# aurianer/DLA-Future

Hardware: AMD Instinct MI355X
Metric: fp64 Cholesky TFlop/s (higher is better)
Workload: dtype f64; 1 GPU; cholesky_d N=65536 nb=1024 uplo=L; grid=1x1, rank_order=column-major, transport=none, work_copies=5

## Files before the change

dla_future_amd/capi.py:

```python
from __future__ import annotations

import ctypes as C
import os

import numpy as np

_HERE = os.path.dirname(os.path.abspath(__file__))


class LibraryNotBuilt(RuntimeError):
    pass


def lib_path() -> str:
    return os.environ.get("DLAF_MI355X_LIB") or os.path.join(_HERE, "lib", "libdlaf_mi355x.so")


class DLAFDescriptor(C.Structure):
    _fields_ = [("m", C.c_int), ("n", C.c_int), ("mb", C.c_int), ("nb", C.c_int), ("isrc", C.c_int),
                ("jsrc", C.c_int), ("i", C.c_int), ("j", C.c_int), ("ld", C.c_int)]


class UpdateDesc(C.Structure):
    _fields_ = ([(n, C.c_long) for n in ("c_elems", "a_elems", "b_elems", "a2_elems", "b2_elems",
                                         "c_off", "a_off", "b_off", "a2_off", "b2_off")] +
                [("tile_layout", C.c_int), ("ltr", C.c_int), ("ltc", C.c_int),
                 ("c_tsr", C.c_long), ("c_tsc", C.c_long), ("ldc", C.c_int),
                 ("a_ts", C.c_long), ("lda", C.c_int),
                 ("b_ts", C.c_long), ("ldb", C.c_int), ("b_period", C.c_int), ("b_ts2", C.c_long), ("b_jl0", C.c_int)] +
                [(n, C.c_int) for n in ("il0", "il1", "jl0", "jl1", "nb", "K", "pr", "ri", "pc", "ci", "nt", "last_rows",
                                        "rect", "nt_c", "last_cols", "K1", "her2k", "info", "role")] +
                [("max_blocks", C.c_long), ("excl_rounds", C.c_int),
                 ("persistent", C.c_long), ("exclusive", C.c_long), ("bulk_slots", C.c_long)])


class TrsmDesc(C.Structure):
    _fields_ = ([(n, C.c_long) for n in ("b_elems", "l_elems", "w_elems", "b_off", "l_off", "w_off", "b_ts")] +
                [(n, C.c_int) for n in ("ldb", "il0", "il1", "pr", "ri", "nb", "nt", "last_rows", "ldl", "n", "upper",
                                        "prio", "info", "winv_source", "unit", "path", "vec", "info_out")])


class PotrfDesc(C.Structure):
    _fields_ = ([(n, C.c_long) for n in ("t_elems", "w_elems", "t_off", "w_off")] +
                [(n, C.c_int) for n in ("kb", "ld", "info", "info_base", "path", "sync_zeroed_by", "count_strips",
                                        "info_out", "t_before_changed", "w_before_changed")])


BCAST_FN = C.CFUNCTYPE(C.c_int, C.c_void_p, C.c_int, C.c_int, C.c_void_p, C.c_size_t)
BARRIER_FN = C.CFUNCTYPE(C.c_int, C.c_void_p)

_TYPE_CHARS = {np.dtype(np.float32): "s", np.dtype(np.float64): "d", np.dtype(np.complex64): "c",
               np.dtype(np.complex128): "z"}


def type_char(dtype) -> str:
    try:
        return _TYPE_CHARS[np.dtype(dtype)]
    except KeyError:
        raise TypeError(f"unsupported element type {dtype}: expected float32/64 or complex64/128") from None


_vp, _i, _l, _ch = C.c_void_p, C.c_int, C.c_long, C.c_char
_IP = C.POINTER(C.c_int)
_i64 = C.c_int64
_LP = C.POINTER(C.c_long)
SIGNATURES = {
    "dlaf_initialize": (None, [_i, C.POINTER(C.c_char_p), _i, C.POINTER(C.c_char_p)]),
    "dlaf_finalize": (None, []),
    "dlaf_free_grid": (None, [_i]),
    "make_dlaf_descriptor": (DLAFDescriptor, [_i, _i, _i, _i, _IP]),
    "dlaf_cholesky_factorization_s": (_i, [_i, _ch, _vp, DLAFDescriptor]),
    "dlaf_cholesky_factorization_d": (_i, [_i, _ch, _vp, DLAFDescriptor]),
    "dlaf_cholesky_factorization_c": (_i, [_i, _ch, _vp, DLAFDescriptor]),
    "dlaf_cholesky_factorization_z": (_i, [_i, _ch, _vp, DLAFDescriptor]),
    "dlaf_pspotrf": (None, [_ch, _i, _vp, _i, _i, _IP, _IP]),
    "dlaf_pdpotrf": (None, [_ch, _i, _vp, _i, _i, _IP, _IP]),
    "dlaf_pcpotrf": (None, [_ch, _i, _vp, _i, _i, _IP, _IP]),
    "dlaf_pzpotrf": (None, [_ch, _i, _vp, _i, _i, _IP, _IP]),
    "dlaf_mi355x_version": (C.c_char_p, []),
    "dlaf_mi355x_create_grid_single": (_i, []),
    "dlaf_mi355x_rccl_unique_id": (None, [_vp]),
    "dlaf_mi355x_create_grid_rccl": (_i, [_vp, _i, _i, _i, _i, _ch]),
    "dlaf_mi355x_create_grid_host": (_i, [_i, _i, _i, _i, _ch, BCAST_FN, BARRIER_FN, _vp]),
    "dlaf_mi355x_grid_host_bcast": (_i, [_i, _i, _i, _vp, C.c_size_t]),
    "dlaf_mi355x_grid_info": (_i, [_i, _IP, _IP, _IP, _IP]),
    "dlaf_mi355x_grid_barrier": (_i, [_i]),
# ... 302 lines not shown
```

dla_future_amd/csrc/device/mma_core.hpp:

```cpp
#pragma once
#include "common.hpp"

namespace dlaf_mi355x {

template <class T, int BM_, int BN_, int WM_, int WN_, int BK_, bool PAIRED_ = false, int STAGES_ = 2,
          int THREADS_ = kThreads>
struct BlockCfg {
  using R = real_t<T>;
  static constexpr bool CX = TypeInfo<T>::is_complex;
  static constexpr int BM = BM_, BN = BN_, WM = WM_, WN = WN_, BK = BK_;
  static constexpr int THREADS = THREADS_, NWAVES = THREADS_ / 64;
  static constexpr int TM = WM / 16, TN = WN / 16;
  static constexpr int WAVES_M = BM / WM, WAVES_N = BN / WN;
  static_assert(WAVES_M * WAVES_N == NWAVES, "the wave tiles must cover the block");
  static_assert(BK % 4 == 0 && WM % 16 == 0 && WN % 16 == 0, "MFMA 16x16x4 granularity");
  static constexpr bool PAIRED = PAIRED_ && !CX;
  static constexpr bool CXI = PAIRED_ && CX;
  static_assert(!PAIRED || (TM % 2 == 0 && TN % 2 == 0), "paired rows: even tile counts");
  static constexpr int PAD = PAIRED_ ? 0 : kLdsPad;
  static constexpr int LDA = BM + PAD, LDB = BN + PAD;
  static constexpr int EPP = CX ? 64 : 1024 / (int) sizeof(T);
  static constexpr int PIECES_A = BK * BM / EPP, PIECES_B = BK * BN / EPP;
  static constexpr bool GLDS =
      (PAIRED && (EPP % BM == 0 || BM % EPP == 0) && (EPP % BN == 0 || BN % EPP == 0) && (BK * BM) % EPP == 0 &&
       (BK * BN) % EPP == 0 && PIECES_A % NWAVES == 0 && PIECES_B % NWAVES == 0) ||
      (CXI && sizeof(T) == 16 && BM % 64 == 0 && BN % 64 == 0 && PIECES_A % NWAVES == 0 && PIECES_B % NWAVES == 0);
  static constexpr int LPS = PIECES_A / NWAVES + PIECES_B / NWAVES;
  static constexpr int A_PLANE = BK * LDA, B_PLANE = BK * LDB;
  static constexpr int A_ELEMS = (CX ? 2 : 1) * A_PLANE, B_ELEMS = (CX ? 2 : 1) * B_PLANE;
  static constexpr int BUF_ELEMS = A_ELEMS + B_ELEMS;
  static constexpr int STAGES = STAGES_;
  static_assert(STAGES >= 2 && STAGES <= 6, "2..6 LDS stages");
  static constexpr int LDS_BYTES = STAGES * BUF_ELEMS * (int) sizeof(R);
};

template <class Cfg>
struct Acc {
  using R = typename Cfg::R;
  using acc_t = typename Mma<R>::acc_t;
  acc_t re[Cfg::TM][Cfg::TN];
  acc_t im[Cfg::CX ? Cfg::TM : 1][Cfg::CX ? Cfg::TN : 1];

  __device__ __forceinline__ void clear() {
#pragma unroll
    for (int i = 0; i < Cfg::TM; ++i)
#pragma unroll
      for (int j = 0; j < Cfg::TN; ++j) {
        re[i][j] = acc_t{0, 0, 0, 0};
        if constexpr (Cfg::CX)
          im[i][j] = acc_t{0, 0, 0, 0};
      }
  }
};

// ... 188 lines not shown
  if constexpr (Cfg::PAIRED)
    return (j >> 1) * 32 + 2 * Mma<R>::irow(g, v) + (j & 1);
  else
    return j * 16 + Mma<R>::irow(g, v);
}

template <class Cfg, class T>
__device__ __forceinline__ void stage_glds(const T* __restrict__ A, long lda, const T* __restrict__ B, long ldb, int k0,
                                           typename Cfg::R* __restrict__ buf, int wave, int lane) {
  constexpr int NA = Cfg::PIECES_A / Cfg::NWAVES, NB = Cfg::PIECES_B / Cfg::NWAVES;
  constexpr int QA0 = 0, QA1 = NA, QB0 = 0, QB1 = NB;
  if constexpr (Cfg::CXI) {
    constexpr int PA = Cfg::BM / 64, PB = Cfg::BN / 64;
#pragma unroll
    for (int idx = QA0; idx < QA1; ++idx) {
      const int piece = wave + Cfg::NWAVES * idx;
      const int k = piece / PA, part = piece % PA;
      const T* ga = A + part * 64 + lane + (long) (k0 + k) * lda;
      __builtin_amdgcn_global_load_lds((const __attribute__((address_space(1))) void*) ga,
                                       (__attribute__((address_space(3))) void*) (buf + 2 * (k * Cfg::LDA + part * 64)),
                                       16, 0, 0);
    }
#pragma unroll
    for (int idx = QB0; idx < QB1; ++idx) {
      const int piece = wave + Cfg::NWAVES * idx;
      const int k = piece / PB, part = piece % PB;
      const T* gb = B + part * 64 + lane + (long) (k0 + k) * ldb;
      __builtin_amdgcn_global_load_lds(
          (const __attribute__((address_space(1))) void*) gb,
          (__attribute__((address_space(3))) void*) (buf + Cfg::A_ELEMS + 2 * (k * Cfg::LDB + part * 64)), 16, 0, 0);
    }
    return;
  }
  constexpr int PER = 16 / (int) sizeof(T);
  constexpr int EPP = Cfg::EPP;
#pragma unroll
  for (int q = QA0; q < QA1; ++q) {
    const int e0 = (wave * NA + q) * EPP;
    const int e = e0 + lane * PER;
    const T* ga = A + (e % Cfg::BM) + (long) (k0 + e / Cfg::BM) * lda;
    __builtin_amdgcn_global_load_lds((const __attribute__((address_space(1))) void*) ga,
                                     (__attribute__((address_space(3))) void*) (buf + e0), 16, 0, 0);
  }
#pragma unroll
  for (int q = QB0; q < QB1; ++q) {
    const int e0 = (wave * NB + q) * EPP;
    const int e = e0 + lane * PER;
    const T* gb = B + (e % Cfg::BN) + (long) (k0 + e / Cfg::BN) * ldb;
    __builtin_amdgcn_global_load_lds((const __attribute__((address_space(1))) void*) gb,
                                     (__attribute__((address_space(3))) void*) (buf + Cfg::A_ELEMS + e0), 16, 0, 0);
  }
}

template <class Cfg, class T, int IDX>
__device__ __forceinline__ void stage_glds_one(const T* __restrict__ A, long lda, const T* __restrict__ B, long ldb,
                                               int k0, typename Cfg::R* __restrict__ buf, int wave, int lane) {
  static_assert(!Cfg::CXI, "real types");
  constexpr int NA = Cfg::PIECES_A / Cfg::NWAVES, NB = Cfg::PIECES_B / Cfg::NWAVES;
  constexpr int PER = 16 / (int) sizeof(T), EPP = Cfg::EPP;
  auto at = [](const T* base, unsigned byte_off) {
    return reinterpret_cast<const T*>(reinterpret_cast<const char*>(base) + byte_off);
  };
  if constexpr (IDX < NA) {
    static_assert(EPP % Cfg::BM == 0 || Cfg::BM % EPP == 0, "pieces and columns nest");
    const int e0 = (wave * NA + IDX) * EPP;
    const unsigned loff = (unsigned) sizeof(T) * (unsigned) ((lane * PER) % Cfg::BM + ((lane * PER) / Cfg::BM) * (int) lda);
    const T* ga = A + (e0 % Cfg::BM) + (long) (k0 + e0 / Cfg::BM) * lda;
    __builtin_amdgcn_global_load_lds((const __attribute__((address_space(1))) void*) at(ga, loff),
                                     (__attribute__((address_space(3))) void*) (buf + e0), 16, 0, 0);
  }
  else if constexpr (IDX < NA + NB) {
    static_assert(EPP % Cfg::BN == 0 || Cfg::BN % EPP == 0, "pieces and columns nest");
    const int e0 = (wave * NB + (IDX - NA)) * EPP;
    const unsigned loff = (unsigned) sizeof(T) * (unsigned) ((lane * PER) % Cfg::BN + ((lane * PER) / Cfg::BN) * (int) ldb);
    const T* gb = B + (e0 % Cfg::BN) + (long) (k0 + e0 / Cfg::BN) * ldb;
    __builtin_amdgcn_global_load_lds((const __attribute__((address_space(1))) void*) at(gb, loff),
                                     (__attribute__((address_space(3))) void*) (buf + Cfg::A_ELEMS + e0), 16, 0, 0);
  }
}

template <class Cfg, class T, bool VEC, bool EDGE, bool UTAIL = false, bool NEG = false>
__device__ __forceinline__ void gemm_nt_block(const T* __restrict__ A, long lda, int mrows,
                                              const T* __restrict__ B, long ldb, int ncols, int K,
                                              typename Cfg::R* __restrict__ lds, Acc<Cfg>& acc, int K1 = 1 << 30,
                                              const T* __restrict__ A2 = nullptr,
                                              const T* __restrict__ B2 = nullptr, int s0 = 0) {
  using R = typename Cfg::R;
  const int lane = threadIdx.x & 63;
  const int wave = __builtin_amdgcn_readfirstlane(threadIdx.x >> 6);
  const int wm = wave % Cfg::WAVES_M, wn = wave / Cfg::WAVES_M;
  const int nk = (K + Cfg::BK - 1) / Cfg::BK;
  if (nk == 0)
    return;
  if constexpr (Cfg::GLDS && VEC && !EDGE) {
    constexpr int ST = Cfg::STAGES;
    constexpr int LPS = Cfg::LPS;
    static_assert(LPS * (ST - 2) < 64, "vmcnt is a 6-bit counter");
#pragma unroll
    for (int s = 0; s < ST - 1; ++s)
      if (s < nk) {
        int sl = s0 + s;
        sl = sl >= nk ? sl - nk : sl;
        stage_glds<Cfg, T>(sl * Cfg::BK < K1 ? A : A2, lda, sl * Cfg::BK < K1 ? B : B2, ldb, sl * Cfg::BK,
                           lds + s * Cfg::BUF_ELEMS, wave, lane);
      }
    if (nk >= ST - 1)
      __builtin_amdgcn_s_waitcnt(0x0070 | ((LPS * (ST - 2)) & 0xF) | ((((LPS * (ST - 2)) >> 4) & 0x3) << 14));
    else
      asm volatile("s_waitcnt vmcnt(0)" ::: "memory");
    __builtin_amdgcn_s_barrier();
    int cur_i = 0, nxt_i = ST - 1;
    constexpr bool SPLIT = !Cfg::CXI && LPS <= (Cfg::BK / 4) * Cfg::TN && LPS <= 16;
    for (int kt = 0; kt < nk; ++kt) {
      R* cur = lds + cur_i * Cfg::BUF_ELEMS;
      const bool load = UTAIL || (kt + ST - 1 < nk);
      int sn = s0 + min(kt + ST - 1, nk - 1);
      sn = sn >= nk ? sn - nk : sn;
      const int kn = sn * Cfg::BK;
      const T* An = kn < K1 ? A : A2;
      const T* Bn = kn < K1 ? B : B2;
      R* nbuf = lds + nxt_i * Cfg::BUF_ELEMS;
      if constexpr (SPLIT) {
        mma_slab<Cfg, NEG>(cur, cur + Cfg::A_ELEMS, acc, wm, wn, lane, [&](int p) {
#define DLAF_GLDS_AT(I)                                                                     \
  if (p == I) {                                                                           \
    if constexpr (I < LPS)                                                                \
      if (load)                                                                           \
        stage_glds_one<Cfg, T, (I < LPS ? I : 0)>(An, lda, Bn, ldb, kn, nbuf, wave, lane); \
  }
          DLAF_GLDS_AT(0) DLAF_GLDS_AT(1) DLAF_GLDS_AT(2) DLAF_GLDS_AT(3) DLAF_GLDS_AT(4) DLAF_GLDS_AT(5)
          DLAF_GLDS_AT(6) DLAF_GLDS_AT(7) DLAF_GLDS_AT(8) DLAF_GLDS_AT(9) DLAF_GLDS_AT(10) DLAF_GLDS_AT(11)
          DLAF_GLDS_AT(12) DLAF_GLDS_AT(13) DLAF_GLDS_AT(14) DLAF_GLDS_AT(15)
#undef DLAF_GLDS_AT
        });
      }
      else {
        if (load)
          stage_glds<Cfg, T>(An, lda, Bn, ldb, kn, nbuf, wave, lane);
        mma_slab<Cfg, NEG>(cur, cur + Cfg::A_ELEMS, acc, wm, wn, lane);
      }
      if (load)
        __builtin_amdgcn_s_waitcnt(0x0070 | ((LPS * (ST - 2)) & 0xF) | ((((LPS * (ST - 2)) >> 4) & 0x3) << 14));
      else
        asm volatile("s_waitcnt vmcnt(0)" ::: "memory");
      asm volatile("s_waitcnt lgkmcnt(0)" ::: "memory");
      __builtin_amdgcn_s_barrier();
      cur_i = (cur_i + 1 == ST) ? 0 : cur_i + 1;
      nxt_i = (nxt_i + 1 == ST) ? 0 : nxt_i + 1;
    }
    if constexpr (UTAIL) {
      asm volatile("s_waitcnt vmcnt(0)" ::: "memory");
      __builtin_amdgcn_s_barrier();
    }
    return;
  }
  Slab<T, Cfg::BM, Cfg::BK, VEC, Cfg::LDA, Cfg::CXI, Cfg::THREADS> sa;
  Slab<T, Cfg::BN, Cfg::BK, VEC, Cfg::LDB, Cfg::CXI, Cfg::THREADS> sb;
  sa.template load<EDGE>(0 < K1 ? A : A2, lda, 0, mrows, K, A2, K1);
  sb.template load<EDGE>(0 < K1 ? B : B2, ldb, 0, ncols, K, B2, K1);
  sa.store(lds);
  sb.store(lds + Cfg::A_ELEMS);
  __syncthreads();
  for (int kt = 0; kt < nk; ++kt) {
    R* cur = lds + (kt & 1) * Cfg::BUF_ELEMS;
    R* nxt = lds + ((kt + 1) & 1) * Cfg::BUF_ELEMS;
    const bool more = (kt + 1) < nk;
    if (more) {
      const int kn = (kt + 1) * Cfg::BK;
      sa.template load<EDGE>(kn < K1 ? A : A2, lda, kn, mrows, K, A2, K1);
      sb.template load<EDGE>(kn < K1 ? B : B2, ldb, kn, ncols, K, B2, K1);
    }
    mma_slab<Cfg, NEG>(cur, cur + Cfg::A_ELEMS, acc, wm, wn, lane);
    if (more) {
      sa.store(nxt);
      sb.store(nxt + Cfg::A_ELEMS);
    }
    __syncthreads();
  }
}

}
```

dla_future_amd/csrc/host/cholesky.cpp:

```cpp
#include "launch_args.hpp"
#include "runtime.hpp"

#include <algorithm>
#include <cstdlib>
#include <cstring>
#include <vector>

namespace dlaf_mi355x {

static bool potrf_use_chain() {
  static const bool chain = [] {
    const char* e = std::getenv("DLAF_MI355X_POTRF");
    return e && std::strcmp(e, "chain") == 0;
  }();
  return chain;
}

template <class T>
void potrf_tile_coop(T* t, int ld, int kb, T* winv, int* info, int info_base, unsigned* sync, hipStream_t s,
                     bool sync_is_zero, bool count_strips) {
  launch_potrf_coop(t, ld, kb, winv, info, info_base, sync, s, sync_is_zero, count_strips);
}

template <class T>
// ... 76 lines not shown
  const long cap = ncols > 0 ? (ncols + period - 1) / period : 0;
  ts2 = cap * (long) tile_elems;
  int issued = 0;
  tr->group_begin();
  for (long c = 0; c < period && c < ncols; ++c) {
    const long jl_first = jl_n + c;
    const long gj_first = cols.global_of(jl_first);
    const int root_r = rows.owner(gj_first);
    long cnt = (ncols - c + period - 1) / period;
    if (cols.global_of(jl_first + (cnt - 1) * period) == nt - 1)
      --cnt;
    if (cnt <= 0)
      continue;
    T* d = dst + c * ts2;
    if (rows.rank == root_r) {
      const T* src = a_base + (size_t) (rows.local_of(gj_first) - il_n) * tile_elems;
      DLAF_HIP_CHECK(hipMemcpy2DAsync(d, tile_bytes, src, (size_t) lstep * tile_bytes, tile_bytes, (size_t) cnt,
                                      hipMemcpyDeviceToDevice, s));
    }
    tr->bcast(ax_col, root_r, rows.rank, d, d, (size_t) cnt * tile_bytes, s);
    ++issued;
  }
  tr->group_end();
  return issued;
}

namespace {

enum class Schedule { Pairs, Sidecar, Early, Classic };

Schedule choose_schedule(bool dist, int nb, bool complex_type) {
  const char* e = std::getenv("DLAF_MI355X_SCHEDULE");
  if (e == nullptr) {
    if (dist)
      return Schedule::Early;
    if (nb % 16 == 0)
      return Schedule::Pairs;
    return !complex_type && nb <= 768 ? Schedule::Sidecar : Schedule::Classic;
  }
  if (std::strcmp(e, "early") == 0)
    return Schedule::Early;
  if (!dist && std::strcmp(e, "pairs") == 0)
    return Schedule::Pairs;
  if (!dist && std::strcmp(e, "sidecar") == 0)
    return Schedule::Sidecar;
  return Schedule::Classic;
}

constexpr long kSidecarSlots = 32;

template <class T>
struct PairRates {
  static constexpr bool dbl = sizeof(real_t<T>) == 8;
  static constexpr double r_bulk = dbl ? 66e12 : 118e12;
  static constexpr double r_trsm_slot = (dbl ? 5e12 : 8e12) / 32.0;
  static constexpr double t_potrf_blk2 = 11.3e-6 * (TypeInfo<T>::is_complex ? 2.0 : 1.0);
};

template <class T>
struct Step {
  const T* a_base = nullptr;
  const T* b_base = nullptr;
  long b_ts = 0, il_n = 0, jl_n = 0;
  int b_period = 1;
  long b_ts2 = 0;
  const T* a2_base = nullptr;
  const T* b2_base = nullptr;
  int k1 = 0;
  int kb = 0;
  long rest0 = 0, split = 0;
  bool valid = false;

  static Step one_panel(int kb, long il_n, long jl_n, const T* a_base, size_t tile_elems) {
    Step st;
    st.valid = true;
    st.kb = kb;
    st.il_n = il_n;
    st.jl_n = jl_n;
    st.a_base = st.b_base = a_base;
    st.b_ts = (long) tile_elems;
    return st;
  }
  static Step two_panels(int k1, int k2, long n0, const T* a_base, const T* a2_base, size_t tile_elems) {
    Step st = one_panel(k1 + k2, n0, n0, a_base, tile_elems);
    st.k1 = k1;
    st.a2_base = st.b2_base = a2_base;
    return st;
  }
};

template <class T>
struct CholeskyIssue {
  using StepT = Step<T>;
  DeviceMatrix<T>& m;
  Transport* tr;
  const bool dist;
  const size_t tile_bytes;
  const CommAxis ax_row, ax_col;
  const hipStream_t s_main, s_panel, s_comm;
  long potrf_slots = 0, comm_slots = 0;
  long grid_reserve = 0;
  size_t next_update_slice = 0;

  explicit CholeskyIssue(DeviceMatrix<T>& mat)
      : m(mat), tr(grid_transport(*mat.grid)), dist(mat.grid->nranks > 1), tile_bytes(mat.tile_elems * sizeof(T)),
        ax_row(mat.transposed ? CommAxis::Col : CommAxis::Row),
        ax_col(mat.transposed ? CommAxis::Row : CommAxis::Col), s_main(mat.s_low), s_panel(mat.s_high),
// ... 491 lines not shown
```

dla_future_amd/csrc/host/update_direct.cpp:

```cpp
#include <algorithm>
#include <vector>

#include <dlaf_mi355x/dlaf_mi355x.h>

#include "launch_args.hpp"
#include "runtime.hpp"
#include "tile_matrix.hpp"

namespace dlaf_mi355x {

namespace {

template <class T>
struct TileGrid {
  T* tiles;
  size_t tile_elems;
  long ltr, ltc;
  int nb;
  Axis rows, cols;
};

template <class T>
struct Operand {
  DevBuf<T> buf;
  T* p = nullptr;
  void put(const void* host, long elems, long off, hipStream_t s) {
    buf.alloc((size_t) (elems + off));
    p = buf.p + off;
    if (elems > 0)
      DLAF_HIP_CHECK(hipMemcpyAsync(p, host, (size_t) elems * sizeof(T), hipMemcpyHostToDevice, s));
  }
};

template <class T>
bool in_bounds(const UpdateArgs<T>& ua, const dlaf_mi355x_update_desc& d) {
  if (ua.pr < 1 || ua.pc < 1 || ua.ri < 0 || ua.ri >= ua.pr || ua.ci < 0 || ua.ci >= ua.pc || ua.il0 < 0 || ua.jl0 < 0 ||
      ua.nb < 1 || ua.K < 1 || ua.nt < 1 || ua.last_rows < 1 || ua.last_rows > ua.nb || ua.ldc < 1 || ua.lda < 1 ||
      ua.ldb < 1 || ua.b_period < 1 || ua.K1 < 0 || ua.K1 >= ua.K || (ua.her2k && ua.K1 == 0) ||
      (ua.rect && (ua.nt_c < 1 || ua.last_cols < 1 || ua.last_cols > ua.nb)) || (ua.rect && ua.her2k))
    return false;
  const int bj0 = ua.b_jl0 >= 0 ? ua.b_jl0 : ua.jl0;
  if (bj0 > ua.jl0)
    return false;
  const long k2 = ua.K - ua.K1;
  const long ka = ua.K1 > 0 ? (ua.her2k ? std::max<long>(ua.K1, k2) : ua.K1) : ua.K;
  const long ka2 = ua.her2k ? std::max<long>(ua.K1, k2) : k2;
  const long kb = ua.K1 > 0 ? ua.K1 : ua.K;
  auto inside = [](long first, long last, long elems) { return first >= 0 && last < elems; };
  for (long il = ua.il0; il < ua.il1; ++il) {
    const long gi = il * ua.pr + ua.ri;
    if (gi >= ua.nt)
      return false;
    const long rows = gi == ua.nt - 1 ? ua.last_rows : ua.nb;
    if (rows > ua.lda || rows > ua.ldc)
      return false;
    const long a0 = (il - ua.il0) * ua.a_ts;
    bool row_used = false;
    for (long jl = ua.jl0; jl < ua.jl1; ++jl) {
      const long gj = jl * ua.pc + ua.ci;
      if (!ua.rect && gi < gj)
        continue;
      if (gj >= (ua.rect ? ua.nt_c : ua.nt))
        return false;
      row_used = true;
      const long cols = ua.rect ? (gj == ua.nt_c - 1 ? ua.last_cols : ua.nb) : (gj == ua.nt - 1 ? ua.last_rows : ua.nb);
      const long c0 = il * ua.c_tsr + jl * ua.c_tsc;
      if (!inside(c0, c0 + rows - 1 + (cols - 1) * ua.ldc, d.c_elems))
        return false;
      if (!ua.rect && gi == gj)
        continue;
      if (cols > ua.ldb)
        return false;
      const long jt = jl - bj0;
      const long b0 = (jt % ua.b_period) * ua.b_ts2 + (jt / ua.b_period) * ua.b_ts;
      if (!inside(b0, b0 + cols - 1 + (kb - 1) * ua.ldb, d.b_elems))
        return false;
      if (ua.K1 > 0 && !inside(b0, b0 + cols - 1 + (k2 - 1) * ua.ldb, d.b2_elems))
        return false;
    }
    if (!row_used)
      continue;
    if (!inside(a0, a0 + rows - 1 + (ka - 1) * ua.lda, d.a_elems))
      return false;
    if (ua.K1 > 0 && !inside(a0, a0 + rows - 1 + (ka2 - 1) * ua.lda, d.a2_elems))
      return false;
  }
  return true;
}

}

template <class T>
long update_bulk_slots() {
  runtime_init();
  hipDeviceProp_t prop;
  int dev = 0;
  DLAF_HIP_CHECK(hipGetDevice(&dev));
  DLAF_HIP_CHECK(hipGetDeviceProperties(&prop, dev));
  return (long) prop.multiProcessorCount * update_blocks_per_cu<T>();
}

template <class T>
int update_direct(dlaf_mi355x_update_desc& d, void* c, const void* a, const void* b, const void* a2, const void* b2,
                  void* c_again) {
  runtime_init();
  if (d.role < 0 || d.role > 4)
    return -1;
  if (d.c_elems < 1 || d.a_elems < 1 || d.b_elems < 1 || d.c_off < 0 || d.a_off < 0 || d.b_off < 0 || d.a2_off < 0 ||
      d.b2_off < 0 || d.excl_rounds < 0 || (d.K1 > 0 && (d.a2_elems < 1 || d.b2_elems < 1 || !a2 || !b2)))
    return -3;
  hipStream_t s = nullptr;
  Operand<T> dc, da, db, da2, db2;
  dc.put(c, d.c_elems, d.c_off, s);
  da.put(a, d.a_elems, d.a_off, s);
  db.put(b, d.b_elems, d.b_off, s);
  if (d.K1 > 0) {
    da2.put(a2, d.a2_elems, d.a2_off, s);
    db2.put(b2, d.b2_elems, d.b2_off, s);
  }
  DevBuf<int> info(1);
  DevBuf<unsigned> counters(16);
  DLAF_HIP_CHECK(hipMemcpyAsync(info.p, &d.info, sizeof(int), hipMemcpyHostToDevice, s));
  DLAF_HIP_CHECK(hipMemsetAsync(counters.p, 0, 16 * sizeof(unsigned), s));

  UpdateArgs<T> ua{};
  if (d.tile_layout) {
    if (d.ltr < 1 || d.ltc < 1 || d.nb < 1 || d.pr < 1 || d.pc < 1 || d.nt < 1)
      return -3;
    TileGrid<T> m;
    m.tiles = dc.p;
    m.tile_elems = (size_t) d.nb * d.nb;
    m.ltr = d.ltr;
    m.ltc = d.ltc;
    m.nb = d.nb;
    m.rows = Axis{(long) (d.nt - 1) * d.nb + d.last_rows, d.nb, d.pr, d.ri, 0};
    m.cols = d.rect ? Axis{(long) (d.nt_c - 1) * d.nb + d.last_cols, d.nb, d.pc, d.ci, 0}
                    : Axis{m.rows.n, d.nb, d.pc, d.ci, 0};
    const T* ap = da.p;
    const T* bp = db.p;
    ua = d.rect ? rect_update_args(m, d.il0, d.il1, d.jl0, d.jl1, ap, bp, d.b_ts, d.K, info.p)
                : update_args(m, d.il0, d.il1, d.jl0, d.jl1, ap, bp, d.b_ts, d.K, info.p);
  }
  else {
    ua.c = dc.p;
    ua.c_tsr = d.c_tsr;
    ua.c_tsc = d.c_tsc;
    ua.ldc = d.ldc;
    ua.a = da.p;
    ua.a_ts = d.a_ts;
    ua.lda = d.lda;
    ua.b = db.p;
    ua.b_ts = d.b_ts;
    ua.ldb = d.ldb;
    ua.il0 = d.il0;
    ua.il1 = d.il1;
    ua.jl0 = d.jl0;
    ua.jl1 = d.jl1;
    ua.nb = d.nb;
    ua.K = d.K;
    ua.pr = d.pr;
    ua.ri = d.ri;
    ua.pc = d.pc;
    ua.ci = d.ci;
    ua.nt = d.nt;
    ua.last_rows = d.last_rows;
    ua.info = info.p;
    ua.rect = d.rect;
    ua.nt_c = d.nt_c;
    ua.last_cols = d.last_cols;
  }
  ua.b_period = d.b_period;
// ... 45 lines not shown
```

include/dlaf_mi355x/dlaf_mi355x.h:

```cpp
#pragma once
#include <stddef.h>
#include <stdint.h>

#include <dlaf_c/desc.h>
#include <dlaf_c/utils.h>

DLAF_EXTERN_C int dlaf_mi355x_create_grid_single(void) DLAF_NOEXCEPT;

#define DLAF_MI355X_UNIQUE_ID_BYTES 128
DLAF_EXTERN_C void dlaf_mi355x_rccl_unique_id(void* out_128_bytes) DLAF_NOEXCEPT;
DLAF_EXTERN_C int dlaf_mi355x_create_grid_rccl(const void* unique_id_128_bytes, int nranks, int rank, int nprow,
                                               int npcol, char order) DLAF_NOEXCEPT;

typedef int (*dlaf_mi355x_bcast_fn)(void* user, int axis, int root, void* host_buf, size_t bytes);
typedef int (*dlaf_mi355x_barrier_fn)(void* user);
DLAF_EXTERN_C int dlaf_mi355x_create_grid_host(int nranks, int rank, int nprow, int npcol, char order,
                                               dlaf_mi355x_bcast_fn bcast, dlaf_mi355x_barrier_fn barrier,
                                               void* user) DLAF_NOEXCEPT;

DLAF_EXTERN_C int dlaf_mi355x_grid_host_bcast(int context, int axis, int root, void* host_buf, size_t bytes) DLAF_NOEXCEPT;

DLAF_EXTERN_C int dlaf_mi355x_grid_on_free(int context, void (*fn)(void*), void* user) DLAF_NOEXCEPT;
DLAF_EXTERN_C int dlaf_mi355x_grid_rekey(int ctx, int new_ctx) DLAF_NOEXCEPT;

// ... 447 lines not shown
DLAF_EXTERN_C int dlaf_mi355x_gmatrix_upload(dlaf_mi355x_gmatrix_t m, const void* host_local, int ld) DLAF_NOEXCEPT;
DLAF_EXTERN_C int dlaf_mi355x_gmatrix_download(dlaf_mi355x_gmatrix_t m, void* host_local, int ld) DLAF_NOEXCEPT;
DLAF_EXTERN_C int dlaf_mi355x_triangular_solver_device(char side, char uplo, char op, char diag, const void* alpha,
                                                       dlaf_mi355x_matrix_t a, dlaf_mi355x_gmatrix_t b) DLAF_NOEXCEPT;
DLAF_EXTERN_C int dlaf_mi355x_potrs_device(char uplo, dlaf_mi355x_matrix_t factor, dlaf_mi355x_gmatrix_t b) DLAF_NOEXCEPT;
DLAF_EXTERN_C int dlaf_mi355x_bt_reduction_to_band_device(int band_size, dlaf_mi355x_gmatrix_t c, dlaf_mi355x_matrix_t v,
                                                          const void* taus) DLAF_NOEXCEPT;

DLAF_EXTERN_C int dlaf_mi355x_solver_profile(double* ms, double* flops) DLAF_NOEXCEPT;

DLAF_EXTERN_C int dlaf_mi355x_triangular_multiplication_device(char side, char uplo, char op, char diag,
                                                               const void* alpha, dlaf_mi355x_matrix_t a,
                                                               dlaf_mi355x_gmatrix_t b) DLAF_NOEXCEPT;
DLAF_EXTERN_C int dlaf_mi355x_hermitian_multiplication_device(char side, char uplo, const void* alpha,
                                                              dlaf_mi355x_matrix_t a, dlaf_mi355x_gmatrix_t b,
                                                              const void* beta, dlaf_mi355x_gmatrix_t c) DLAF_NOEXCEPT;
DLAF_EXTERN_C int dlaf_mi355x_multiplication_profile(double* ms, double* flops) DLAF_NOEXCEPT;

DLAF_EXTERN_C int dlaf_mi355x_set_random_hpd(int context, char type, void* host_local,
                                             struct DLAF_descriptor desc, int nthreads) DLAF_NOEXCEPT;

DLAF_EXTERN_C int dlaf_mi355x_tile_potrf(char type, char uplo, int n, void* a, int lda) DLAF_NOEXCEPT;
DLAF_EXTERN_C int dlaf_mi355x_tile_trsm(char type, char uplo, int m, int n, const void* a, int lda, void* b,
                                        int ldb) DLAF_NOEXCEPT;
DLAF_EXTERN_C int dlaf_mi355x_tile_herk(char type, char uplo, int n, int k, const void* a, int lda, void* c,
                                        int ldc) DLAF_NOEXCEPT;
DLAF_EXTERN_C int dlaf_mi355x_tile_gemm(char type, char uplo, int m, int n, int k, const void* a, int lda,
                                        const void* b, int ldb, void* c, int ldc) DLAF_NOEXCEPT;

struct dlaf_mi355x_update_desc {
  long c_elems, a_elems, b_elems, a2_elems, b2_elems;
  long c_off, a_off, b_off, a2_off, b2_off;
  int tile_layout, ltr, ltc;
  long c_tsr, c_tsc;
  int ldc;
  long a_ts;
  int lda;
  long b_ts;
  int ldb;
  int b_period;
  long b_ts2;
  int b_jl0;
  int il0, il1, jl0, jl1, nb, K;
  int pr, ri, pc, ci;
  int nt, last_rows;
  int rect, nt_c, last_cols;
  int K1, her2k;
  int info;
  int role;
  long max_blocks;
  int excl_rounds;
  long persistent, exclusive;
  long bulk_slots;
};
DLAF_EXTERN_C int dlaf_mi355x_update_direct_s(struct dlaf_mi355x_update_desc* d, void* c, const void* a, const void* b,
                                              const void* a2, const void* b2, void* c_again) DLAF_NOEXCEPT;
DLAF_EXTERN_C int dlaf_mi355x_update_direct_d(struct dlaf_mi355x_update_desc* d, void* c, const void* a, const void* b,
                                              const void* a2, const void* b2, void* c_again) DLAF_NOEXCEPT;
DLAF_EXTERN_C int dlaf_mi355x_update_direct_c(struct dlaf_mi355x_update_desc* d, void* c, const void* a, const void* b,
                                              const void* a2, const void* b2, void* c_again) DLAF_NOEXCEPT;
DLAF_EXTERN_C int dlaf_mi355x_update_direct_z(struct dlaf_mi355x_update_desc* d, void* c, const void* a, const void* b,
                                              const void* a2, const void* b2, void* c_again) DLAF_NOEXCEPT;
DLAF_EXTERN_C long dlaf_mi355x_update_bulk_slots(char type) DLAF_NOEXCEPT;

DLAF_EXTERN_C int dlaf_mi355x_triangular_inverse_s(int context, char uplo, char diag, float* a,
                                                   struct DLAF_descriptor desca) DLAF_NOEXCEPT;
DLAF_EXTERN_C int dlaf_mi355x_inverse_from_cholesky_factor_s(int context, char uplo, float* a,
                                                             struct DLAF_descriptor desca) DLAF_NOEXCEPT;
DLAF_EXTERN_C void dlaf_mi355x_pstrtri(char uplo, char diag, int n, float* a, int ia, int ja, const int desca[9],
                                       int* info) DLAF_NOEXCEPT;
DLAF_EXTERN_C void dlaf_mi355x_pspotri(char uplo, int n, float* a, int ia, int ja, const int desca[9],
                                       int* info) DLAF_NOEXCEPT;
DLAF_EXTERN_C int dlaf_mi355x_triangular_inverse_d(int context, char uplo, char diag, double* a,
                                                   struct DLAF_descriptor desca) DLAF_NOEXCEPT;
DLAF_EXTERN_C int dlaf_mi355x_inverse_from_cholesky_factor_d(int context, char uplo, double* a,
                                                             struct DLAF_descriptor desca) DLAF_NOEXCEPT;
DLAF_EXTERN_C void dlaf_mi355x_pdtrtri(char uplo, char diag, int n, double* a, int ia, int ja, const int desca[9],
                                       int* info) DLAF_NOEXCEPT;
DLAF_EXTERN_C void dlaf_mi355x_pdpotri(char uplo, int n, double* a, int ia, int ja, const int desca[9],
                                       int* info) DLAF_NOEXCEPT;
DLAF_EXTERN_C int dlaf_mi355x_triangular_inverse_c(int context, char uplo, char diag, dlaf_complex_c* a,
                                                   struct DLAF_descriptor desca) DLAF_NOEXCEPT;
DLAF_EXTERN_C int dlaf_mi355x_inverse_from_cholesky_factor_c(int context, char uplo, dlaf_complex_c* a,
                                                             struct DLAF_descriptor desca) DLAF_NOEXCEPT;
DLAF_EXTERN_C void dlaf_mi355x_pctrtri(char uplo, char diag, int n, dlaf_complex_c* a, int ia, int ja, const int desca[9],
                                       int* info) DLAF_NOEXCEPT;
DLAF_EXTERN_C void dlaf_mi355x_pcpotri(char uplo, int n, dlaf_complex_c* a, int ia, int ja, const int desca[9],
                                       int* info) DLAF_NOEXCEPT;
DLAF_EXTERN_C int dlaf_mi355x_triangular_inverse_z(int context, char uplo, char diag, dlaf_complex_z* a,
                                                   struct DLAF_descriptor desca) DLAF_NOEXCEPT;
DLAF_EXTERN_C int dlaf_mi355x_inverse_from_cholesky_factor_z(int context, char uplo, dlaf_complex_z* a,
                                                             struct DLAF_descriptor desca) DLAF_NOEXCEPT;
DLAF_EXTERN_C void dlaf_mi355x_pztrtri(char uplo, char diag, int n, dlaf_complex_z* a, int ia, int ja, const int desca[9],
                                       int* info) DLAF_NOEXCEPT;
DLAF_EXTERN_C void dlaf_mi355x_pzpotri(char uplo, int n, dlaf_complex_z* a, int ia, int ja, const int desca[9],
                                       int* info) DLAF_NOEXCEPT;
DLAF_EXTERN_C int dlaf_mi355x_triangular_inverse_device(char uplo, char diag, dlaf_mi355x_matrix_t m) DLAF_NOEXCEPT;
DLAF_EXTERN_C int dlaf_mi355x_inverse_from_cholesky_factor_device(char uplo, dlaf_mi355x_matrix_t m) DLAF_NOEXCEPT;
DLAF_EXTERN_C int dlaf_mi355x_inverse_profile(double* ms, double* flops) DLAF_NOEXCEPT;
DLAF_EXTERN_C int dlaf_mi355x_inverse_plan(long n, int nb, int nprow, int npcol, int myrow, int mycol, int isrc,
                                           int jsrc, long out[9]) DLAF_NOEXCEPT;
DLAF_EXTERN_C int dlaf_mi355x_inverse_step(long n, int nb, int nprow, int npcol, int myrow, int mycol, int isrc,
                                           int jsrc, long k, long out[7]) DLAF_NOEXCEPT;

DLAF_EXTERN_C int dlaf_mi355x_general_norm_s(int context, char norm, const float* a, struct DLAF_descriptor desca,
                                             double* value) DLAF_NOEXCEPT;
// ... 101 lines not shown
```

Before: 70.55 TFlop/s.

## Precompute global-to-LDS piece addresses incrementally in split GEMM pipeline

Replaces the per-piece global_load_lds address computation with a per-wave base pointer and a fixed per-lane offset. The base is advanced by compile-time step sizes between pieces and computed once at the first hook, and the per-iteration load flag becomes a compile-time constant when UTAIL is set. The goal is fewer integer address instructions interleaved with the MFMA slab. It also retunes the fp64 real bulk rate used by the Cholesky scheduler and adds a test-path option to place second operands below the first in one allocation. The scheduler rate change can alter the work split between kernels.

```diff
diff --git a/dla_future_amd/capi.py b/dla_future_amd/capi.py
--- a/dla_future_amd/capi.py
+++ b/dla_future_amd/capi.py
@@ -31,7 +31,8 @@
                 [(n, C.c_int) for n in ("il0", "il1", "jl0", "jl1", "nb", "K", "pr", "ri", "pc", "ci", "nt", "last_rows",
                                         "rect", "nt_c", "last_cols", "K1", "her2k", "info", "role")] +
                 [("max_blocks", C.c_long), ("excl_rounds", C.c_int),
-                 ("persistent", C.c_long), ("exclusive", C.c_long), ("bulk_slots", C.c_long)])
+                 ("persistent", C.c_long), ("exclusive", C.c_long), ("bulk_slots", C.c_long),
+                 ("second_below", C.c_int)])
 
 
 class TrsmDesc(C.Structure):
diff --git a/dla_future_amd/csrc/device/glds_addr.hpp b/dla_future_amd/csrc/device/glds_addr.hpp
--- /dev/null
+++ b/dla_future_amd/csrc/device/glds_addr.hpp
@@ -0,0 +1,43 @@
+#pragma once
+
+#if defined(__HIPCC__)
+#define DLAF_GLDS_HD __host__ __device__
+#else
+#define DLAF_GLDS_HD
+#endif
+
+namespace dlaf_mi355x {
+
+DLAF_GLDS_HD constexpr int glds_slab_ahead(int kt, int ahead, int nk, int s0) {
+  const int t = kt + ahead < nk - 1 ? kt + ahead : nk - 1;
+  const int sn = s0 + t;
+  return sn >= nk ? sn - nk : sn;
+}
+
+template <int ROWS, int EPP, int N, int ELEM_BYTES>
+struct GldsPieces {
+  static constexpr int CPP = EPP >= ROWS ? EPP / ROWS : 1;
+  static constexpr int PPC = EPP >= ROWS ? 1 : ROWS / EPP;
+  static constexpr int PER = 16 / ELEM_BYTES;
+  static_assert(EPP >= ROWS ? EPP % ROWS == 0 : (ROWS % EPP == 0 && N % PPC == 0),
+                "pieces and columns nest, and a wave's run of pieces starts at the top of a column");
+  static_assert(EPP == 64 * PER, "one piece = 64 lanes x 16 bytes");
+
+  static DLAF_GLDS_HD constexpr long long base_elems(int wave, int k0, long long ld) {
+    const unsigned column = (unsigned) (k0 + wave * (N / PPC) * CPP);
+    return (long long) ((unsigned long long) column * (unsigned long long) (unsigned) ld);
+  }
+  static DLAF_GLDS_HD constexpr long long step_bytes(int idx, long long ld) {
+    if (EPP >= ROWS)
+      return (long long) ELEM_BYTES * CPP * ld;
+    return (long long) ELEM_BYTES * (idx % PPC == 0 ? ld - (long long) (PPC - 1) * EPP : (long long) EPP);
+  }
+  static DLAF_GLDS_HD constexpr unsigned lane_bytes(int lane, long long ld) {
+    return (unsigned) ELEM_BYTES * ((unsigned) ((lane * PER) % ROWS) + (unsigned) ((lane * PER) / ROWS) * (unsigned) ld);
+  }
+  static DLAF_GLDS_HD constexpr bool lane_fits(long long ld) {
+    return (long long) ELEM_BYTES * ((CPP - 1) * ld + ROWS) <= 0x7fffffffLL;
+  }
+};
+
+}
diff --git a/dla_future_amd/csrc/device/mma_core.hpp b/dla_future_amd/csrc/device/mma_core.hpp
--- a/dla_future_amd/csrc/device/mma_core.hpp
+++ b/dla_future_amd/csrc/device/mma_core.hpp
@@ -1,5 +1,8 @@
 #pragma once
+#include <type_traits>
+
 #include "common.hpp"
+#include "glds_addr.hpp"
 
 namespace dlaf_mi355x {
 
@@ -294,31 +297,16 @@
   }
 }
 
-template <class Cfg, class T, int IDX>
-__device__ __forceinline__ void stage_glds_one(const T* __restrict__ A, long lda, const T* __restrict__ B, long ldb,
-                                               int k0, typename Cfg::R* __restrict__ buf, int wave, int lane) {
-  static_assert(!Cfg::CXI, "real types");
-  constexpr int NA = Cfg::PIECES_A / Cfg::NWAVES, NB = Cfg::PIECES_B / Cfg::NWAVES;
-  constexpr int PER = 16 / (int) sizeof(T), EPP = Cfg::EPP;
-  auto at = [](const T* base, unsigned byte_off) {
-    return reinterpret_cast<const T*>(reinterpret_cast<const char*>(base) + byte_off);
-  };
-  if constexpr (IDX < NA) {
-    static_assert(EPP % Cfg::BM == 0 || Cfg::BM % EPP == 0, "pieces and columns nest");
-    const int e0 = (wave * NA + IDX) * EPP;
-    const unsigned loff = (unsigned) sizeof(T) * (unsigned) ((lane * PER) % Cfg::BM + ((lane * PER) / Cfg::BM) * (int) lda);
-    const T* ga = A + (e0 % Cfg::BM) + (long) (k0 + e0 / Cfg::BM) * lda;
-    __builtin_amdgcn_global_load_lds((const __attribute__((address_space(1))) void*) at(ga, loff),
-                                     (__attribute__((address_space(3))) void*) (buf + e0), 16, 0, 0);
-  }
-  else if constexpr (IDX < NA + NB) {
-    static_assert(EPP % Cfg::BN == 0 || Cfg::BN % EPP == 0, "pieces and columns nest");
-    const int e0 = (wave * NB + (IDX - NA)) * EPP;
-    const unsigned loff = (unsigned) sizeof(T) * (unsigned) ((lane * PER) % Cfg::BN + ((lane * PER) / Cfg::BN) * (int) ldb);
-    const T* gb = B + (e0 % Cfg::BN) + (long) (k0 + e0 / Cfg::BN) * ldb;
-    __builtin_amdgcn_global_load_lds((const __attribute__((address_space(1))) void*) at(gb, loff),
-                                     (__attribute__((address_space(3))) void*) (buf + Cfg::A_ELEMS + e0), 16, 0, 0);
-  }
+template <class R>
+__device__ __forceinline__ void glds_load_piece(const char* piece, unsigned& lane_off, R* dst) {
+  asm volatile("" : "+v"(lane_off));
+  __builtin_amdgcn_global_load_lds((const __attribute__((address_space(1))) void*) (piece + lane_off),
+                                   (__attribute__((address_space(3))) void*) dst, 16, 0, 0);
+}
+
+template <class Cfg>
+__device__ __host__ constexpr int glds_hook_of(int i) {
+  return kRotatedSlab<Cfg> ? i + 1 : i;
 }
 
 template <class Cfg, class T, bool VEC, bool EDGE, bool UTAIL = false, bool NEG = false>
@@ -353,42 +341,83 @@
     __builtin_amdgcn_s_barrier();
     int cur_i = 0, nxt_i = ST - 1;
     constexpr bool SPLIT = !Cfg::CXI && LPS <= (Cfg::BK / 4) * Cfg::TN && LPS <= 16;
-    for (int kt = 0; kt < nk; ++kt) {
-      R* cur = lds + cur_i * Cfg::BUF_ELEMS;
-      const bool load = UTAIL || (kt + ST - 1 < nk);
-      int sn = s0 + min(kt + ST - 1, nk - 1);
-      sn = sn >= nk ? sn - nk : sn;
-      const int kn = sn * Cfg::BK;
-      const T* An = kn < K1 ? A : A2;
-      const T* Bn = kn < K1 ? B : B2;
-      R* nbuf = lds + nxt_i * Cfg::BUF_ELEMS;
-      if constexpr (SPLIT) {
-        mma_slab<Cfg, NEG>(cur, cur + Cfg::A_ELEMS, acc, wm, wn, lane, [&](int p) {
-#define DLAF_GLDS_AT(I)                                                                     \
-  if (p == I) {                                                                           \
-    if constexpr (I < LPS)                                                                \
-      if (load)                                                                           \
-        stage_glds_one<Cfg, T, (I < LPS ? I : 0)>(An, lda, Bn, ldb, kn, nbuf, wave, lane); \
-  }
-          DLAF_GLDS_AT(0) DLAF_GLDS_AT(1) DLAF_GLDS_AT(2) DLAF_GLDS_AT(3) DLAF_GLDS_AT(4) DLAF_GLDS_AT(5)
-          DLAF_GLDS_AT(6) DLAF_GLDS_AT(7) DLAF_GLDS_AT(8) DLAF_GLDS_AT(9) DLAF_GLDS_AT(10) DLAF_GLDS_AT(11)
-          DLAF_GLDS_AT(12) DLAF_GLDS_AT(13) DLAF_GLDS_AT(14) DLAF_GLDS_AT(15)
-#undef DLAF_GLDS_AT
-        });
-      }
-      else {
+    if constexpr (!SPLIT) {
+      for (int kt = 0; kt < nk; ++kt) {
+        R* cur = lds + cur_i * Cfg::BUF_ELEMS;
+        const bool load = UTAIL || (kt + ST - 1 < nk);
+        int sn = s0 + min(kt + ST - 1, nk - 1);
+        sn = sn >= nk ? sn - nk : sn;
+        const int kn = sn * Cfg::BK;
+        const T* An = kn < K1 ? A : A2;
+        const T* Bn = kn < K1 ? B : B2;
+        R* nbuf = lds + nxt_i * Cfg::BUF_ELEMS;
         if (load)
           stage_glds<Cfg, T>(An, lda, Bn, ldb, kn, nbuf, wave, lane);
         mma_slab<Cfg, NEG>(cur, cur + Cfg::A_ELEMS, acc, wm, wn, lane);
-      }
-      if (load)
-        __builtin_amdgcn_s_waitcnt(0x0070 | ((LPS * (ST - 2)) & 0xF) | ((((LPS * (ST - 2)) >> 4) & 0x3) << 14));
-      else
-        asm volatile("s_waitcnt vmcnt(0)" ::: "memory");
-      asm volatile("s_waitcnt lgkmcnt(0)" ::: "memory");
-      __builtin_amdgcn_s_barrier();
-      cur_i = (cur_i + 1 == ST) ? 0 : cur_i + 1;
-      nxt_i = (nxt_i + 1 == ST) ? 0 : nxt_i + 1;
+        if (load)
+          __builtin_amdgcn_s_waitcnt(0x0070 | ((LPS * (ST - 2)) & 0xF) | ((((LPS * (ST - 2)) >> 4) & 0x3) << 14));
+        else
+          asm volatile("s_waitcnt vmcnt(0)" ::: "memory");
+        asm volatile("s_waitcnt lgkmcnt(0)" ::: "memory");
+        __builtin_amdgcn_s_barrier();
+        cur_i = (cur_i + 1 == ST) ? 0 : cur_i + 1;
+        nxt_i = (nxt_i + 1 == ST) ? 0 : nxt_i + 1;
+      }
+    }
+    else {
+      constexpr int NA = Cfg::PIECES_A / Cfg::NWAVES, NB = Cfg::PIECES_B / Cfg::NWAVES;
+      using PA = GldsPieces<Cfg::BM, Cfg::EPP, NA, (int) sizeof(T)>;
+      using PB = GldsPieces<Cfg::BN, Cfg::EPP, NB, (int) sizeof(T)>;
+      unsigned lane_a = PA::lane_bytes(lane, lda), lane_b = PB::lane_bytes(lane, ldb);
+      auto iteration = [&](int kt, auto load) {
+        R* cur = lds + cur_i * Cfg::BUF_ELEMS;
+        R* nbuf = lds + nxt_i * Cfg::BUF_ELEMS;
+        {
+          const char* pa = nullptr;
+          const char* pb = nullptr;
+          mma_slab<Cfg, NEG>(cur, cur + Cfg::A_ELEMS, acc, wm, wn, lane, [&](int p) {
+            if (p == glds_hook_of<Cfg>(0)) {
+              const int kn = glds_slab_ahead(kt, ST - 1, nk, s0) * Cfg::BK;
+              pa = reinterpret_cast<const char*>((kn < K1 ? A : A2) + PA::base_elems(wave, kn, lda));
+              pb = reinterpret_cast<const char*>((kn < K1 ? B : B2) + PB::base_elems(wave, kn, ldb));
+            }
+#define DLAF_GLDS_AT(I)                                                                              \
+  if constexpr (I < LPS)                                                                             \
+    if (p == glds_hook_of<Cfg>(I)) {                                                                 \
+      if constexpr (I < NA) {                                                                        \
+        if (load)                                                                                    \
+          glds_load_piece(pa, lane_a, nbuf + (wave * NA + I) * Cfg::EPP);                            \
+        if constexpr (I + 1 < NA)                                                                    \
+          pa += PA::step_bytes(I + 1, lda);                                                          \
+      }                                                                                              \
+      else {                                                                                         \
+        if (load)                                                                                    \
+          glds_load_piece(pb, lane_b, nbuf + Cfg::A_ELEMS + (wave * NB + (I - NA)) * Cfg::EPP);      \
+        if constexpr (I + 1 < LPS)                                                                   \
+          pb += PB::step_bytes(I + 1 - NA, ldb);                                                     \
+      }                                                                                              \
+    }
+            DLAF_GLDS_AT(0) DLAF_GLDS_AT(1) DLAF_GLDS_AT(2) DLAF_GLDS_AT(3) DLAF_GLDS_AT(4) DLAF_GLDS_AT(5)
+            DLAF_GLDS_AT(6) DLAF_GLDS_AT(7) DLAF_GLDS_AT(8) DLAF_GLDS_AT(9) DLAF_GLDS_AT(10) DLAF_GLDS_AT(11)
+            DLAF_GLDS_AT(12) DLAF_GLDS_AT(13) DLAF_GLDS_AT(14) DLAF_GLDS_AT(15)
+#undef DLAF_GLDS_AT
+          });
+        }
+        if (load)
+          __builtin_amdgcn_s_waitcnt(0x0070 | ((LPS * (ST - 2)) & 0xF) | ((((LPS * (ST - 2)) >> 4) & 0x3) << 14));
+        else
+          asm volatile("s_waitcnt vmcnt(0)" ::: "memory");
+        asm volatile("s_waitcnt lgkmcnt(0)" ::: "memory");
+        __builtin_amdgcn_s_barrier();
+        cur_i = (cur_i + 1 == ST) ? 0 : cur_i + 1;
+        nxt_i = (nxt_i + 1 == ST) ? 0 : nxt_i + 1;
+      };
+      for (int kt = 0; kt < nk; ++kt) {
+        if constexpr (UTAIL)
+          iteration(kt, std::true_type{});
+        else
+          iteration(kt, kt + ST - 1 < nk);
+      }
     }
     if constexpr (UTAIL) {
       asm volatile("s_waitcnt vmcnt(0)" ::: "memory");
diff --git a/dla_future_amd/csrc/host/cholesky.cpp b/dla_future_amd/csrc/host/cholesky.cpp
--- a/dla_future_amd/csrc/host/cholesky.cpp
+++ b/dla_future_amd/csrc/host/cholesky.cpp
@@ -152,7 +152,7 @@
 template <class T>
 struct PairRates {
   static constexpr bool dbl = sizeof(real_t<T>) == 8;
-  static constexpr double r_bulk = dbl ? 66e12 : 118e12;
+  static constexpr double r_bulk = dbl ? (TypeInfo<T>::is_complex ? 66e12 : 70e12) : 118e12;
   static constexpr double r_trsm_slot = (dbl ? 5e12 : 8e12) / 32.0;
   static constexpr double t_potrf_blk2 = 11.3e-6 * (TypeInfo<T>::is_complex ? 2.0 : 1.0);
 };
diff --git a/dla_future_amd/csrc/host/update_direct.cpp b/dla_future_amd/csrc/host/update_direct.cpp
--- a/dla_future_amd/csrc/host/update_direct.cpp
+++ b/dla_future_amd/csrc/host/update_direct.cpp
@@ -29,6 +29,15 @@
     p = buf.p + off;
     if (elems > 0)
       DLAF_HIP_CHECK(hipMemcpyAsync(p, host, (size_t) elems * sizeof(T), hipMemcpyHostToDevice, s));
+  }
+  void put_below(const void* host, long elems, long off, Operand& hi, const void* hi_host, long hi_elems, long hi_off,
+                 hipStream_t s) {
+    const long span = (off + elems + 15) / 16 * 16;
+    buf.alloc((size_t) (span + hi_off + hi_elems));
+    p = buf.p + off;
+    hi.p = buf.p + span + hi_off;
+    DLAF_HIP_CHECK(hipMemcpyAsync(p, host, (size_t) elems * sizeof(T), hipMemcpyHostToDevice, s));
+    DLAF_HIP_CHECK(hipMemcpyAsync(hi.p, hi_host, (size_t) hi_elems * sizeof(T), hipMemcpyHostToDevice, s));
   }
 };
 
@@ -112,11 +121,17 @@
   hipStream_t s = nullptr;
   Operand<T> dc, da, db, da2, db2;
   dc.put(c, d.c_elems, d.c_off, s);
-  da.put(a, d.a_elems, d.a_off, s);
-  db.put(b, d.b_elems, d.b_off, s);
-  if (d.K1 > 0) {
-    da2.put(a2, d.a2_elems, d.a2_off, s);
-    db2.put(b2, d.b2_elems, d.b2_off, s);
+  if (d.K1 > 0 && d.second_below) {
+    da2.put_below(a2, d.a2_elems, d.a2_off, da, a, d.a_elems, d.a_off, s);
+    db2.put_below(b2, d.b2_elems, d.b2_off, db, b, d.b_elems, d.b_off, s);
+  }
+  else {
+    da.put(a, d.a_elems, d.a_off, s);
+    db.put(b, d.b_elems, d.b_off, s);
+    if (d.K1 > 0) {
+      da2.put(a2, d.a2_elems, d.a2_off, s);
+      db2.put(b2, d.b2_elems, d.b2_off, s);
+    }
   }
   DevBuf<int> info(1);
   DevBuf<unsigned> counters(16);
diff --git a/include/dlaf_mi355x/dlaf_mi355x.h b/include/dlaf_mi355x/dlaf_mi355x.h
--- a/include/dlaf_mi355x/dlaf_mi355x.h
+++ b/include/dlaf_mi355x/dlaf_mi355x.h
@@ -523,6 +523,7 @@
   int excl_rounds;
   long persistent, exclusive;
   long bulk_slots;
+  int second_below;
 };
 DLAF_EXTERN_C int dlaf_mi355x_update_direct_s(struct dlaf_mi355x_update_desc* d, void* c, const void* a, const void* b,
                                               const void* a2, const void* b2, void* c_again) DLAF_NOEXCEPT;
```

After: 71.92 TFlop/s, median of 6. 1.9% higher.
